# amcpherson/remixt

Measured on AMD Instinct MI355X. Metric: EM iterations/sec (50k seg x 165 states), higher is better.
Workload: dtype f64

## Files before the change

include/remixt_amd.h:

```cpp
#ifndef REMIXT_AMD_H
#define REMIXT_AMD_H

#include <stdint.h>

#ifdef __cplusplus
extern "C" {
#endif

#define RMX_OK 0
#define RMX_EVALUE 1
#define RMX_EASSERT 2
#define RMX_EDEVICE 3
#define RMX_EUNSUPPORTED 4
#define RMX_EARG 5

#define RMX_MAX_CLONES 4

typedef struct rmx_batch rmx_batch;

typedef struct rmx_problem {
    int32_t num_clones;
    int32_t num_segments;
    int32_t num_breakpoints;
    int32_t num_cn_states;
// ... 57 lines not shown
    RMX_OPT_VITERBI_PLAIN,
    RMX_OPT_SEARCH_MODE,
    RMX_OPT_ELL_DENSE,
    RMX_OPT_STRIP,
    RMX_OPT_CELL_CACHE,
    RMX_OPT_SPARSE_TRIAL,
    RMX_OPT_FB_DEBUG,
    RMX_OPT_PAIRWISE_KERNEL,
    RMX_OPT_PACE_SWEEPS,
    RMX_OPT_FB_WG_BUDGET,
    RMX_OPT_TRIAL_KERNEL,
    RMX_OPT_GRAD_KERNEL,
    RMX_OPT_STREAM_POOL,
    RMX_OPT_VITERBI_CLUSTER,
    RMX_OPT_TRACEBACK,
    RMX_OPT_COUNT
};
int rmx_set_default_option(int32_t option_id, int32_t value);
int rmx_set_option(rmx_batch *b, int32_t option_id, int32_t value);
int rmx_get_option(rmx_batch *b, int32_t option_id, int32_t *value);

int rmx_set_param(rmx_batch *b, int32_t r, int32_t param_id, double value);
int rmx_get_param(rmx_batch *b, int32_t r, int32_t param_id, double *value);
int rmx_set_transition_model(rmx_batch *b, int32_t model);
int rmx_set_array(rmx_batch *b, int32_t r, int32_t array_id, const void *host_src);
int rmx_get_array(rmx_batch *b, int32_t r, int32_t array_id, void *host_dst);
int rmx_fetch_indicators(rmx_batch *b, int32_t r0, int32_t r1, const double **total, const double **allele);
int rmx_calculate_log_transmat(rmx_batch *b, int32_t r, double *dst);
int rmx_weighted_search(const double *p, int64_t n, const double *u, int32_t k, int64_t *out, int64_t *positive);
int rmx_weighted_sample_round(const double *w, int64_t n, int64_t stride, double norm, const double *u, int32_t k,
// ... 74 lines not shown
```

remixt_amd/bpmodel.py:

```python
import ctypes as C

import numpy as np

from . import _lib

_dp = C.POINTER(C.c_double)
_ip = C.POINTER(C.c_int64)
_i32p = C.POINTER(C.c_int32)

RMX_EVALUE, RMX_EASSERT, RMX_EDEVICE, RMX_EUNSUPPORTED, RMX_EARG = 1, 2, 3, 4, 5

MAX_CLONES = 4
PARAM_IDS = {
    'negbin_r_0': 0, 'negbin_r_1': 1, 'negbin_hdel_mu': 2, 'negbin_hdel_r_0': 3, 'negbin_hdel_r_1': 4,
    'betabin_M_0': 5, 'betabin_M_1': 6, 'betabin_loh_p': 7, 'betabin_loh_M_0': 8, 'betabin_loh_M_1': 9,
    'prior_outlier_total': 10, 'prior_outlier_allele': 11, 'divergence_weight': 12, 'hmm_log_norm_const': 13,
}
ARRAY_IDS = {
    'h': 0, 'p_breakpoint': 1, 'p_allele_swap': 2, 'p_outlier_total': 3, 'p_outlier_allele': 4,
    'posterior_marginals': 5, 'framelogprob': 6, 'total_likelihood_mask': 7, 'allele_likelihood_mask': 8,
    'log_transmat': 9, 'cached_log_transmat': 10, 'joint_posterior_marginals': 11, 'state_sequence': 12,
}
_WRITABLE = {'h', 'p_breakpoint', 'p_allele_swap', 'p_outlier_total', 'p_outlier_allele', 'posterior_marginals',
             'total_likelihood_mask', 'allele_likelihood_mask'}
_STATE_TABLES = {'cn_states_total': 0, 'num_alleles_subclonal': 1, 'is_hdel': 2, 'is_loh': 3}


OPTION_IDS = dict((n, i) for i, n in enumerate((
    'fb_kernel', 'fb_nv', 'fb_breakend_codes', 'fuse_sweeps', 'two_streams', 'viterbi_plain', 'search_mode', 'ell_dense', 'strip',
    'cell_cache', 'sparse_trial', 'fb_debug', 'pairwise_kernel', 'pace_sweeps', 'fb_wg_budget', 'trial_kernel', 'grad_kernel', 'stream_pool', 'viterbi_cluster', 'traceback')))


def set_default_option(name, value):
    lib = _lib.load()
    rc = lib.rmx_set_default_option(OPTION_IDS[name], int(value))
    if rc:
        _raise(lib, rc)


def last_error_restarts():
    lib = _lib.load()
    n = lib.rmx_last_error_restarts(None, 0)
    if n <= 0:
        return []
    buf = (C.c_int32 * n)()
# ... 791 lines not shown
```

remixt_amd/csrc/rmx_api.hip:

```cpp
#include <hip/hip_runtime.h>
#include <algorithm>
#include <cmath>
#include <limits>
#include <atomic>
#include <cstdio>
#include <cstring>
#include <functional>
#include <map>
#include <mutex>
#include <string>
#include <vector>
#include <chrono>
#include <cstdlib>
#include <condition_variable>
#include <memory>

#include "rmx_kernels.h"
#include "rmx_host.h"

static thread_local std::string g_err;
static thread_local std::vector<int32_t> g_err_restarts;
static int fail(int code, const std::string &msg) { g_err = msg; g_err_restarts.clear(); return code; }
static int fail_flagged(int code, const std::string &msg) { g_err = msg; return code; }
static inline long long now_ns() { return std::chrono::duration_cast<std::chrono::nanoseconds>(std::chrono::steady_clock::now().time_since_epoch()).count(); }
// ... 21 lines not shown
    StreamPool &p = g_stream_pool[dev & 15];
    std::lock_guard<std::mutex> lk(p.mu);
    std::vector<hipStream_t> &idle = p.idle[role];
    if (!idle.empty()) { *out = idle.front(); idle.erase(idle.begin()); return RMX_OK; }
    if (hipStreamCreateWithFlags(out, hipStreamNonBlocking) != hipSuccess) return RMX_EDEVICE;
    p.created[role]++;
    return RMX_OK;
}
static void pool_release(int dev, int role, hipStream_t s) {
    hipStreamSynchronize(s);
    StreamPool &p = g_stream_pool[dev & 15];
    std::lock_guard<std::mutex> lk(p.mu);
    p.idle[role].push_back(s);
}

static int g_opt_default[RMX_OPT_COUNT] = {0, 0, 1, 1, 1, 0, 5, 0, 1, 1, 1, 0, 0, 0, 0, 0, 0, 1, 0, 0};
static std::mutex g_opt_mu;

struct rmx_batch {
    hipEvent_t ev_pace = nullptr;
    int opt[RMX_OPT_COUNT];
    int device = 0;
    hipStream_t stream = nullptr;
    hipStream_t stream2 = nullptr;
    hipEvent_t ev_fb = nullptr, ev_brk = nullptr;
    bool own_stream = false, pooled_stream = false, pooled_stream2 = false;
    Dev d{};
    int R = 0;
    std::vector<int64_t> cn_classes;
    std::vector<int32_t> seg_class, brk_idx, brk_orient, tclass, brk_slot, be_n;
    std::vector<int64_t> brk_states, is_telomere;
// ... 455 lines not shown
                for (int k = 0; k < 8; k++) b->segc_built[(size_t)q * 8 + k] = b->rp[q].p[ids[k]];
                return true;
            };
            if (!stale(r)) { r++; continue; }
            int e = r + 1;
            while (e < r1 && stale(e)) e++;
            { ProfScope ps(b, KID_SEG_CONST); hipLaunchKernelGGL(k_seg_const, dim3((b->d.N + 255) / 256, e - r), dim3(256), 0, b->stream, b->d, r); }
            for (int i = r; i < e; i++) b->segc_dirty[i] = 0;
            r = e;
        }
    }
    HIPCHK(hipGetLastError());
    return RMX_OK;
}
typedef void (*cells_kernel_t)(Dev, int);
template <int NS> static cells_kernel_t cells_kernel_ns(int mode, int mask, int cache) {
    if (mode == 0) return cache == 2 ? k_cells<NS, 0, CM_ALL, 2> : (cache == 1 ? k_cells<NS, 0, CM_ALL, 1> : k_cells<NS, 0, CM_ALL, 0>);
    if (mode == 1) return cache == 2 ? k_cells<NS, 1, CM_ALL, 2> : k_cells<NS, 1, CM_ALL, 0>;
    if (mode == 3) return k_cells<NS, 3, CM_ALL, 2>;
    if (cache == 2) return k_cells<NS, 2, 31, 2>;
    if (cache == 1) {
        switch (mask) {
        case 1: return k_cells<NS, 2, 1, 1>; case 2: return k_cells<NS, 2, 2, 1>;
        case 3: return k_cells<NS, 2, 3, 1>; case 4: return k_cells<NS, 2, 4, 1>; case 8: return k_cells<NS, 2, 8, 1>;
        case 12: return k_cells<NS, 2, 12, 1>; case 15: return k_cells<NS, 2, 15, 1>; default: return k_cells<NS, 2, 31, 1>;
        }
    }
    switch (mask) {
    case 1: return k_cells<NS, 2, 1, 0>; case 2: return k_cells<NS, 2, 2, 0>;
    case 3: return k_cells<NS, 2, 3, 0>; case 4: return k_cells<NS, 2, 4, 0>; case 8: return k_cells<NS, 2, 8, 0>;
    case 12: return k_cells<NS, 2, 12, 0>; case 15: return k_cells<NS, 2, 15, 0>; default: return k_cells<NS, 2, 31, 0>;
    }
}
static bool use_strip(rmx_batch *b) { return b->d.S > 32 && b->d.S <= 384 && b->opt[RMX_OPT_STRIP]; }
static cells_kernel_t cells_kernel(rmx_batch *b, int mode, int mask, int cache) {
    const int ns = (b->d.S + 63) / 64;
    switch (ns) { case 1: return cells_kernel_ns<1>(mode, mask, cache); case 2: return cells_kernel_ns<2>(mode, mask, cache);
                  case 3: return cells_kernel_ns<3>(mode, mask, cache); case 4: return cells_kernel_ns<4>(mode, mask, cache);
                  case 5: return cells_kernel_ns<5>(mode, mask, cache); default: return cells_kernel_ns<6>(mode, mask, cache); }
}
static dim3 ell_block(rmx_batch *b) { return dim3(std::min(256, ((b->d.S + 63) / 64) * 64)); }
static bool ell_sparse_ok(rmx_batch *b, int n, const int32_t *restarts) {
    if (!b->d.sig_cnt || b->opt[RMX_OPT_ELL_DENSE]) return false;
    for (int i = 0; i < n; i++) if (!b->sig_valid[restarts[i]]) return false;
    return true;
}
static dim3 strip_grid(rmx_batch *b, int nr) { return dim3((b->d.N + 4 * STRIP_RPW - 1) / (4 * STRIP_RPW), nr); }
static int cover_mask(int m) {
    if (m & 16) return 31;
    if ((m & 3) && (m & 12)) return 15;
    if ((m & 3) == 3) return 3;
    if (m & 1) return 1;
    if (m & 2) return 2;
    if ((m & 12) == 12) return 12;
// ... 176 lines not shown
    case RMX_OPT_VITERBI_CLUSTER: return v == 0 || v == 1 || v == 2 || v == 4 || v == 8 || v == 102 || v == 104 || v == 108;
    case RMX_OPT_TRACEBACK: return v == 0 || v == 1;
    case RMX_OPT_VITERBI_PLAIN: return v >= 0 && v <= 2;
    default: return v == 0 || v == 1;
    }
}
int rmx_set_default_option(int32_t id, int32_t value) {
    if (id < 0 || id >= RMX_OPT_COUNT || !option_value_ok(id, value)) return fail(RMX_EARG, "bad option id / value");
    std::lock_guard<std::mutex> lk(g_opt_mu);
    g_opt_default[id] = value;
    return RMX_OK;
}
static void configure_fb(rmx_batch *b);
int rmx_set_option(rmx_batch *b, int32_t id, int32_t value) {
    if (!b || id < 0 || id >= RMX_OPT_COUNT || !option_value_ok(id, value)) return fail(RMX_EARG, "bad option id / value");
    if (id == RMX_OPT_CELL_CACHE || id == RMX_OPT_SPARSE_TRIAL || id == RMX_OPT_FB_DEBUG || id == RMX_OPT_STREAM_POOL) return fail(RMX_EARG, "creation-time option: use rmx_set_default_option before rmx_batch_create");
    BIND(b);
    b->opt[id] = value;
    if (id == RMX_OPT_FB_KERNEL) configure_fb(b);
    return RMX_OK;
}
int rmx_get_option(rmx_batch *b, int32_t id, int32_t *value) {
    if (!b || !value || id < 0 || id >= RMX_OPT_COUNT) return fail(RMX_EARG, "bad option id");
    BIND(b);
    *value = b->opt[id];
    return RMX_OK;
}

int rmx_compress_cn_states(const int64_t *cn_states, int32_t N, int32_t S, int32_t M, int32_t max_classes,
                           int32_t *seg_class_out, int64_t *classes_out, int32_t *num_classes) {
    const int rc = rmxh::compress_cn_states(cn_states, N, S, M, max_classes, seg_class_out, classes_out, num_classes);
// ... 157 lines not shown
        if (M == 4 && d.D <= 21 && d.NBE > 0) {
            b->pe2p = (d.D * d.D * d.D + 1) & ~1;
            DA(pe2_lt, double, (size_t)R * d.NBE * b->pe2p + 2)
        }
    }
    if ((rc = dalloc(b, &b->d_A2, RN * 2)) || (rc = dalloc(b, &b->d_Bv2, RN * 4))) { rmx_batch_destroy(b); return rc; }
    if ((rc = dalloc(b, &b->d_cnpack, (size_t)C * S)) || (rc = dalloc(b, &b->d_cnpack2, (size_t)C * S)) || (rc = dalloc(b, &b->d_totpack, (size_t)C * S)) || (rc = dalloc(b, &b->d_wk, (size_t)std::max(d.TC, 1) * FBK_WKN))) { rmx_batch_destroy(b); return rc; }
    DA(pd_cached, double, BEW) DA(hist, double, BEW) DA(be_jt, double, (size_t)R * d.NBE) DA(be_ja, double, (size_t)R * d.NBE)
    DA(err, uint32_t, R)
#undef DA
    d.lc = nullptr; d.sig_idx = nullptr; d.sig_cnt = nullptr;
    if (S > 32 && S <= 384 && b->opt[RMX_OPT_SPARSE_TRIAL]) {
        uint16_t *pi_ = nullptr; uint8_t *pc_ = nullptr;
        if (dalloc(b, &pi_, RN * RMX_SIGK) == RMX_OK && dalloc(b, &pc_, RN) == RMX_OK) { d.sig_idx = pi_; d.sig_cnt = pc_; }
    }
    {
        const size_t bytes = RNS * 6 * 8;
        const bool want = b->opt[RMX_OPT_CELL_CACHE] != 0;
        if (want && S > 32 && S <= 384 && bytes <= ((size_t)96 << 30)) { double *p_ = nullptr; if (dalloc(b, &p_, RNS * 6) == RMX_OK) { d.lc = p_; b->use_cache = true; } }
    }
    if ((rc = dalloc(b, &b->d_lt_valid, R)) || (rc = dalloc(b, &b->d_partial, (size_t)R * ELBO_BLOCKS * 5)) || (rc = dalloc(b, &b->d_be_e, (size_t)R * std::max(d.NBE, 1))) || (rc = dalloc(b, &b->d_out4, (size_t)R * 5)) ||
        (rc = dalloc(b, &b->d_ell_partial, (size_t)R * std::max(N, ELBO_BLOCKS) * (1 + RMX_MAX_CLONES))) || (rc = dalloc(b, &b->d_ell_out, (size_t)R * 8)) ||
        (rc = dalloc(b, &b->d_sample, (size_t)R * N)) || (rc = dalloc(b, &b->d_grid_out, (size_t)R * 64 * (1 + RMX_MAX_CLONES))) ||
        (rc = dalloc(b, &b->d_done, std::max(R, 64))) || (rc = dalloc(b, &b->d_rlist, R)) || (rc = dalloc(b, &b->d_counts, R)) || (rc = dalloc(b, &b->d_rp_stage, R)) || (rc = dalloc(b, &b->d_batch_out, (size_t)R * 8))) { rmx_batch_destroy(b); return rc; }
    HIPCHK(hipMemset(b->d_done, 0, sizeof(unsigned) * (size_t)std::max(R, 64)));
    HIPCHK(hipHostMalloc((void **)&b->h_pinned, sizeof(double) * (size_t)(R + 1) * 64 * (1 + RMX_MAX_CLONES)));
    HIPCHK(hipHostMalloc((void **)&b->h_err, sizeof(uint32_t) * ((size_t)R * 4 + 64)));
    HIPCHK(hipHostMalloc(&b->h_batch, (size_t)R * (sizeof(RestartParams) + 64) + 4096));
    HIPCHK(hipEventCreate(&b->tm_a)); HIPCHK(hipEventCreate(&b->tm_b));
    b->done_ev.resize(R);
    for (int r = 0; r < R; r++) HIPCHK(hipEventCreateWithFlags(&b->done_ev[r], hipEventDisableTiming));

    if ((rc = build_transitions(b))) { rmx_batch_destroy(b); return rc; }
    {
// ... 85 lines not shown
    if (b->own_stream) { if (b->pooled_stream) pool_release(b->device, 0, b->stream); else hipStreamDestroy(b->stream); b->own_stream = false; b->pooled_stream = false; }
    if (s) b->stream = (hipStream_t)s;
    else { HIPCHK(hipStreamCreateWithFlags(&b->stream, hipStreamNonBlocking)); b->own_stream = true; }
    return RMX_OK;
}
int rmx_synchronize(rmx_batch *b) { BIND(b); HIPCHK(hipStreamSynchronize(b->stream)); return RMX_OK; }

int rmx_info(rmx_batch *b, int32_t what, int64_t *out) { BIND(b);
    switch (what) {
    case 0: *out = b->d.cn_max; break; case 1: *out = b->d.NC; break; case 2: *out = b->d.TC; break; case 3: *out = b->d.NBE; break;
    case 4: *out = b->d.SP; break; case 5: *out = b->fbv_rpt; break; case 6: *out = b->fbG.P; break; case 7: *out = b->fbG.NT; break;
    case 8: *out = b->fbG.BLK; break; case 9: *out = (int64_t)b->fbG_lds; break; case 10: *out = b->n_fast; break; case 11: *out = b->n_generic; break;
    case 60: *out = b->t_launch_ns; break; case 61: *out = b->t_wait_ns; break; case 62: *out = b->t_post_ns; break; case 63: *out = b->n_rounds; break;
    case 12: *out = b->last_fb_kernel; break; case 13: *out = b->last_fb_nv; break; case 14: *out = b->last_viterbi; break; case 15: *out = b->last_fb_nv_max; break;
    case 18: *out = b->last_viterbi_wgs; break; case 19: *out = b->last_traceback; break;
    case 54: *out = b->cluster_timeouts; break;
    case 52: *out = b->last_search_blocks; break;
    case 16: { StreamPool &p_ = g_stream_pool[b->device & 15]; std::lock_guard<std::mutex> lk(p_.mu); *out = p_.created[0] + p_.created[1]; break; }
    case 17: { StreamPool &p_ = g_stream_pool[b->device & 15]; std::lock_guard<std::mutex> lk(p_.mu); *out = (int64_t)(p_.idle[0].size() + p_.idle[1].size()); break; }
    case 20: case 21: case 22: case 23: case 24: case 25: case 26: case 27: case 28: case 29: case 30: case 31: case 32: case 33: case 34: case 35: case 36: case 37: case 38: case 39:
    case 40: case 41: case 42: case 43: case 44: case 45: case 46: case 47: case 48: case 49: case 50: case 51:
        { if (!b->d_dbg) { *out = 0; break; } unsigned long long v[32]; HIPCHK(hipStreamSynchronize(b->stream)); HIPCHK(hipMemcpy(v, b->d_dbg, 256, hipMemcpyDeviceToHost)); *out = (int64_t)v[what - 20]; break; }
    default: return fail(RMX_EARG, "bad info id");
    }
    return RMX_OK;
}

static const int kParamComponents[RMX_P_HMM_LOG_NORM_CONST] = {CM_LT0, CM_LT1, CM_LT0 | CM_LT1, CM_LT0, CM_LT1, CM_LA0, CM_LA1, CM_LA0 | CM_LA1, CM_LA0, CM_LA1, 0, 0, 16};
int rmx_set_param(rmx_batch *b, int32_t r, int32_t id, double v) { BIND(b);
    if (r < 0 || r >= b->R || id < 0 || id >= RMX_P_HMM_LOG_NORM_CONST) return fail(RMX_EARG, "bad restart / param id");
// ... 1253 lines not shown
    for (int i = 0; i < nr; i++) out[i] = b->h_pinned[i];
    return RMX_OK;
}

static int trial_pass(rmx_batch *b, int r0, int r1, Dev &d2) {
    b->trial_comp_r0 = b->trial_comp_r1 = -1;
    b->scratch_r0 = b->scratch_r1 = -1;
    int rc = ensure_tables(b, r0, r1);
    if (rc) return rc;
    const Dev &d = b->d;
    const int nr = r1 - r0;
    const size_t RN0 = (size_t)r0 * d.N, cnt = (size_t)nr * d.N;
    HIPCHK(hipMemcpyAsync(b->d_A2 + RN0 * 2, d.A + RN0 * 2, cnt * 16, hipMemcpyDeviceToDevice, b->stream));
    HIPCHK(hipMemcpyAsync(b->d_Bv2 + RN0 * 4, d.Bv + RN0 * 4, cnt * 32, hipMemcpyDeviceToDevice, b->stream));
    d2 = b->d;
    d2.A = b->d_A2; d2.Bv = b->d_Bv2; d2.lc = nullptr;
    for (int r = r0; r < r1;) {
        const int mask = use_strip(b) ? cover_mask(b->comp_dirty[r] & 15) : (b->comp_dirty[r] ? 15 : 0);
        int e = r + 1;
        while (e < r1 && (use_strip(b) ? cover_mask(b->comp_dirty[e] & 15) : (b->comp_dirty[e] ? 15 : 0)) == mask) e++;
        if (mask) {
            ProfScope ps(b, KID_MARGINALS_AB);
            bool sparse = use_strip(b) && d.sig_cnt != nullptr;
            for (int i = r; i < e; i++) if (!b->sig_valid[i]) sparse = false;
            if (sparse) {
                void (*kf)(Dev, int) = nullptr;
                if (b->opt[RMX_OPT_TRIAL_KERNEL] == 0) {
                    switch (mask) {
                    case 1: kf = k_trial_flat<1>; break; case 2: kf = k_trial_flat<2>; break; case 3: kf = k_trial_flat<3>; break;
                    case 4: kf = k_trial_flat<4>; break; case 8: kf = k_trial_flat<8>; break; case 12: kf = k_trial_flat<12>; break;
                    default: kf = k_trial_flat<15>; break;
// ... 559 lines not shown
```

remixt_amd/csrc/rmx_device.h:

```cpp
#pragma once
#include <hip/hip_runtime.h>
#include <stdint.h>
#include "../../include/remixt_amd.h"

#define RMX_ERR_NAN_LL 1u
#define RMX_ERR_BAD_P 2u
#define RMX_ERR_TOTAL_DEPTH 4u
#define RMX_ERR_LOH_P 8u
#define RMX_ERR_NAN_F 16u
#define RMX_ERR_NAN_AB 32u
#define RMX_ERR_NAN_POST 64u
#define RMX_ERR_DIGAMMA 128u
#define RMX_ERR_NAN_GRAD 256u

#define ST_HDEL_NB 1u
#define ST_LOH_M 2u
#define ST_E_TD 4u
#define ST_E_LOH 8u
#define ST_E_BADP 16u
#define ST_GZ_ALLELE 32u

struct RestartParams {
    double h[RMX_MAX_CLONES];
    double p[RMX_P_COUNT];
// ... 26 lines not shown
    const int8_t *af, *ab;
    const uint16_t *pcode;
    const int32_t *jord, *jmeta;
    RestartParams *rp;
    double *stD, *stP, *stM, *stLg;
    double *stLogD;
    uint32_t *stFlags;
    uint32_t *stFlagsAgg;
    double *segc;
    double *qt, *qa, *qs;
    double *pbrk;
    double *f, *fe, *fa, *fb, *post;
    double *fe_alt;
    uint16_t *sig_idx; uint8_t *sig_cnt;
    double *lc;
    double *fmax, *mrow;
    double *A, *Bv;
    double *rowPF, *rowPP, *rowZ;
    double *pd_lt, *pd_cached;
    double *pe_lt;
    double *pe2_lt;
    double *pe2x_lt;
    double *hist;
    double *be_jt, *be_ja;
    uint32_t *err;
};

__device__ __forceinline__ size_t rs_off(const Dev &d, int r, int n) { return ((size_t)r * d.N + n) * d.SP; }

__device__ __forceinline__ double g_transition(int tmodel, int cn_diff) {
// ... 339 lines not shown
```

remixt_amd/csrc/rmx_host.h:

```cpp
#ifndef RMX_HOST_H
#define RMX_HOST_H
#include <algorithm>
#include <cmath>
#include <cstdint>
#include <cstring>
#include <vector>

#if defined(__HIPCC__)
#define RMX_HD __host__ __device__
#else
#define RMX_HD
#endif

namespace rmxh {

inline int compress_cn_states(const int64_t *cn_states, int32_t N, int32_t S, int32_t M, int32_t max_classes,
                              int32_t *seg_class_out, int64_t *classes_out, int32_t *num_classes) {
    if (!cn_states || !seg_class_out || !classes_out || !num_classes) return 5;
    const size_t tsz = (size_t)S * M * 2;
    int C = 0;
    for (int n = 0; n < N; n++) {
        const int64_t *t = cn_states + (size_t)n * tsz;
        int found = -1;
        if (n > 0 && memcmp(t, classes_out + (size_t)seg_class_out[n - 1] * tsz, tsz * 8) == 0) found = seg_class_out[n - 1];
        for (int c = 0; c < C && found < 0; c++) if (memcmp(t, classes_out + (size_t)c * tsz, tsz * 8) == 0) found = c;
        if (found < 0) {
            if (C >= max_classes) return 4;
            memcpy(classes_out + (size_t)C * tsz, t, tsz * 8);
            found = C++;
        }
        seg_class_out[n] = found;
    }
    *num_classes = C;
    return 0;
}

inline int weighted_search(const double *p, int64_t n, const double *u, int32_t k, int64_t *out, int64_t *positive) {
    if (!p || n < 1 || (k > 0 && (!u || !out))) return 5;
    std::vector<double> cdf((size_t)n);
    double acc = 0.;
    int64_t pos = 0;
    for (int64_t i = 0; i < n; i++) { acc += p[i]; cdf[(size_t)i] = acc; pos += p[i] > 0.; }
    const double last = cdf[(size_t)n - 1];
    for (int64_t i = 0; i < n; i++) cdf[(size_t)i] /= last;
    for (int32_t j = 0; j < k; j++) {
        const int64_t idx = (int64_t)(std::upper_bound(cdf.begin(), cdf.end(), u[j]) - cdf.begin());
        out[j] = std::min<int64_t>(idx, n - 1);
    }
// ... 111 lines not shown
```

remixt_amd/csrc/rmx_kernels.h:

```cpp
#pragma once
#include "rmx_device.h"
#include "rmx_host.h"
#define SEGL 32
#define SEG_PER_BLOCK (256 / SEGL)
#define TRIAL_SEGL 16
#define RMX_CLUSTER_SPINS (1u << 22)
#define FBK_WKN 128
#define NM_MAX_SAMPLE 1024
#define TRIAL_SEG_PER_BLOCK (256 / TRIAL_SEGL)


__device__ __forceinline__ void state_tables_body(const Dev &d, int cls, int r, const RestartParams &rp) {
    __shared__ unsigned agg_sh;
    if (threadIdx.x == 0) agg_sh = 0u;
    __syncthreads();
    unsigned agg = 0u;
    for (int s = threadIdx.x; s < d.S; s += blockDim.x) {
        const int8_t *cn = d.cn + ((size_t)cls * d.S + s) * d.M * 2;
        const int8_t *tot = d.tot + ((size_t)cls * d.S + s) * d.M;
        double minor = 0., total = 0.;
        for (int m = 0; m < d.M; m++) {
            minor += rp.h[m] * (double)cn[m * 2 + 0];
            total += rp.h[m] * (double)tot[m];
        }
// ... 1588 lines not shown
    }
    a0 = group_sum(a0, G); a1 = group_sum(a1, G);
    b0 = group_sum(b0, G); b1 = group_sum(b1, G); b2 = group_sum(b2, G); b3 = group_sum(b3, G);
    pf = group_sum(pf, G); pp = group_sum(pp, G);
    if (gl == 0) {
        const size_t rn = (size_t)r * d.N + n;
        d.A[rn * 2] = a0; d.A[rn * 2 + 1] = a1;
        d.Bv[rn * 4] = b0; d.Bv[rn * 4 + 1] = b1; d.Bv[rn * 4 + 2] = b2; d.Bv[rn * 4 + 3] = b3;
        d.rowPF[rn] = pf; d.rowPP[rn] = pp;
        if (COMPUTE_POST) d.rowZ[rn] = d.fmax[rn] + (d.chain_end_flag[n] ? log(sum) : log(d.mrow[rn]));
    }
    if (err) atomicOr(&d.err[r], err);
}

#define STRIP_RPW 8
template <int NS, int MODE, int MASK, int CACHE>
__global__ __launch_bounds__(256) void k_cells(Dev d, int r0) {
    const int r = r0 + blockIdx.y;
    const int lane = threadIdx.x & 63;
    const int wave = __builtin_amdgcn_readfirstlane((int)(threadIdx.x >> 6));
    const int nbeg = (blockIdx.x * 4 + wave) * STRIP_RPW;
    if (nbeg >= d.N) return;
    const int nend = min(d.N, nbeg + STRIP_RPW);
    const RestartParams &rp = d.rp[r];
    const int S = d.S;
    StateRegs st[NS];
    int cur_cls = -1;
    auto nsub_of = [&](int cls_, int s_) { return (double)((d.sflags[(size_t)cls_ * d.S + s_] >> 2) & 3); };
    unsigned err = 0;
    const double divw = rp.p[RMX_P_DIVERGENCE_WEIGHT];
    const size_t plane = (size_t)d.N * d.SP;
    double *lcr = d.lc ? d.lc + (size_t)r * 6 * plane : nullptr;
    auto cell = [&](const SegCtx &sc, const StateRegs &stx, size_t off, double LT[2], double LA[4]) {
        if (CACHE == 2) {
            LT[0] = lcr[off]; LT[1] = lcr[plane + off];
            LA[0] = lcr[2 * plane + off]; LA[1] = lcr[3 * plane + off]; LA[2] = lcr[4 * plane + off]; LA[3] = lcr[5 * plane + off];
        } else {
            cell_ll_regs<MASK & CM_ALL>(rp, sc, stx, LT, LA, err);
            if (CACHE == 1) {
                if (MASK & CM_LT0) lcr[off] = LT[0];
                if (MASK & CM_LT1) lcr[plane + off] = LT[1];
                if (MASK & CM_LA0) { lcr[2 * plane + off] = LA[0]; lcr[3 * plane + off] = LA[1]; }
                if (MASK & CM_LA1) { lcr[4 * plane + off] = LA[2]; lcr[5 * plane + off] = LA[3]; }
            }
        }
    };
    double lp_prior[4] = {0., 0., 0., 0.};
    if (MODE == 3) {
        const double pt_ = rp.p[RMX_P_PRIOR_OUTLIER_TOTAL], pa_ = rp.p[RMX_P_PRIOR_OUTLIER_ALLELE];
        lp_prior[0] = log_prior(1. - pt_); lp_prior[1] = log_prior(pt_); lp_prior[2] = log_prior(1. - pa_); lp_prior[3] = log_prior(pa_);
    }
    constexpr bool PREFETCH = (MODE == 1 || MODE == 3) && NS >= 2 && NS <= 4;
    double pfa[PREFETCH ? NS : 1], pfb[PREFETCH ? NS : 1];
    if (PREFETCH) {
        const size_t ro0 = ((size_t)r * d.N + nbeg) * d.SP;
#pragma unroll
        for (int k = 0; k < NS; k++) { const int s = lane + 64 * k; pfa[k] = s < S ? d.fa[ro0 + s] : 0.; pfb[k] = s < S ? d.fb[ro0 + s] : 0.; }
    }
    for (int n = nbeg; n < nend; n++) {
        const int cls = d.seg_class[n];
        if (CACHE != 2 && cls != cur_cls) {
#pragma unroll
            for (int k = 0; k < NS; k++) { const int s = lane + 64 * k; load_state_regs(d, r, cls, s < S ? s : S - 1, st[k]); }
            cur_cls = cls;
        }
        SegCtx sc; load_seg(d, r, n, sc);
        const size_t rn = (size_t)r * d.N + n;
        const size_t ro = rn * d.SP;
        if (MODE == 0) {
            const double qt0 = d.qt[rn * 2], qt1 = d.qt[rn * 2 + 1], qa0 = d.qa[rn * 2], qa1 = d.qa[rn * 2 + 1];
            const double qs0 = d.qs[rn * 2], qs1 = d.qs[rn * 2 + 1];
            double fv[NS];
            double vmax = -INFINITY;
#pragma unroll
            for (int k = 0; k < NS; k++) {
                const int s = lane + 64 * k;
                fv[k] = -INFINITY;
                if (s < S) {
                    double LT[2], LA[4];
                    cell(sc, st[k], (size_t)n * d.SP + s, LT, LA);
                    double f = 0.;
                    f += qt0 * LT[0]; f += qt1 * LT[1];
                    f += qa0 * qs0 * LA[0]; f += qa0 * qs1 * LA[1]; f += qa1 * qs0 * LA[2]; f += qa1 * qs1 * LA[3];
                    f += -1.0 * (CACHE == 2 ? nsub_of(cls, s) : st[k].nsub) * sc.l * divw;
                    if (f != f) err |= RMX_ERR_NAN_F;
                    d.f[ro + s] = f;
                    fv[k] = f;
                    vmax = fmax(vmax, f);
                }
                __builtin_amdgcn_sched_barrier(0);
            }
            vmax = group_max(vmax, 64);
            if (lane == 0) d.fmax[rn] = vmax;
#pragma unroll
            for (int k = 0; k < NS; k++) { const int s = lane + 64 * k; if (s < d.SP) d.fe[ro + s] = s < S ? exp_fast(fv[k] - vmax) : 0.; }
        } else {
            constexpr bool M1 = MODE == 1 || MODE == 3;
            constexpr int NSTASH = MODE != 3 ? 0 : (NS <= 3 ? 6 : (NS <= 6 ? 3 : 0));
            constexpr bool STASH = NSTASH > 0;
            __shared__ double lsm[STASH ? 4 : 1][STASH ? NS * NSTASH * 64 : 1];
            double pv[NS];
            double sum = 0.;
            if (M1) {
#pragma unroll
                for (int k = 0; k < NS; k++) {
                    const int s = lane + 64 * k;
                    pv[k] = PREFETCH ? pfa[PREFETCH ? k : 0] * pfb[PREFETCH ? k : 0] : (s < S ? d.fa[ro + s] * d.fb[ro + s] : 0.);
                    sum += pv[k];
                }
                if (PREFETCH && n + 1 < nend) {
#pragma unroll
                    for (int k = 0; k < NS; k++) { const int s = lane + 64 * k; pfa[PREFETCH ? k : 0] = s < S ? d.fa[ro + d.SP + s] : 0.; pfb[PREFETCH ? k : 0] = s < S ? d.fb[ro + d.SP + s] : 0.; }
                }
// ... 13 lines not shown
                        const bool sg_ = s < S && pv[k] >= RMX_POST_EPS;
                        const unsigned long long bal_ = __ballot(sg_);
                        const int pos_ = base_ + __popcll(bal_ & ((1ull << lane) - 1ull));
                        if (sg_ && pos_ < RMX_SIGK) d.sig_idx[rn * RMX_SIGK + pos_] = (uint16_t)s;
                        base_ += __popcll(bal_);
                    }
                    if (lane == 0) d.sig_cnt[rn] = base_ <= RMX_SIGK ? (uint8_t)base_ : (uint8_t)255;
                }
            } else {
#pragma unroll
                for (int k = 0; k < NS; k++) { const int s = lane + 64 * k; pv[k] = s < S ? d.post[ro + s] : 0.; }
            }
            double a0 = 0., a1 = 0., b0 = 0., b1 = 0., b2 = 0., b3 = 0., pf = 0., pp = 0.;
            double fq[6] = {0., 0., 0., 0., 0., 0.};
            if (MODE == 1) { fq[0] = d.qt[rn * 2]; fq[1] = d.qt[rn * 2 + 1]; fq[2] = d.qa[rn * 2]; fq[3] = d.qa[rn * 2 + 1]; fq[4] = d.qs[rn * 2]; fq[5] = d.qs[rn * 2 + 1]; }
#pragma unroll
            for (int k = 0; k < NS; k++) {
                const int s = lane + 64 * k;
                if (MODE == 2 && CACHE == 0 && !(MASK & 16) && !__any(pv[k] >= RMX_POST_EPS)) { if (s < S) cell_static_errors<MASK & CM_ALL>(sc, st[k].fl, err); continue; }
                if (s < S) {
                    double LT[2], LA[4];
                    cell(sc, st[k], (size_t)n * d.SP + s, LT, LA);
                    const double ps = pv[k];
                    if (STASH) {
#pragma unroll
                        for (int q_ = 0; q_ < 2; q_++) if (q_ < NSTASH) lsm[wave][(k * NSTASH + q_) * 64 + lane] = LT[q_];
#pragma unroll
                        for (int q_ = 0; q_ < 4; q_++) if (2 + q_ < NSTASH) lsm[wave][(k * NSTASH + 2 + q_) * 64 + lane] = LA[q_];
                    }
                    a0 += ps * LT[0]; a1 += ps * LT[1];
                    b0 += ps * LA[0]; b1 += ps * LA[1]; b2 += ps * LA[2]; b3 += ps * LA[3];
                    if (MODE == 1) {
                        double f = 0.;
                        f += fq[0] * LT[0]; f += fq[1] * LT[1];
                        f += fq[2] * fq[4] * LA[0]; f += fq[2] * fq[5] * LA[1]; f += fq[3] * fq[4] * LA[2]; f += fq[3] * fq[5] * LA[3];
                        f += -1.0 * (CACHE == 2 ? nsub_of(cls, s) : st[k].nsub) * sc.l * divw;
                        d.f[ro + s] = f;
                        pf += ps * f;
                    }
                    if (MODE == 2 && (MASK & 16)) pf += ps * d.f[ro + s];
                    if (MODE == 1 || (MODE == 2 && (MASK & 16))) pp += ps * (-1.0 * (CACHE == 2 ? nsub_of(cls, s) : st[k].nsub) * sc.l * divw);
                }
                __builtin_amdgcn_sched_barrier(0);
// ... 39 lines not shown
                { const double ss_ = qs0 + qs1; qs0 /= ss_; qs1 /= ss_; }
                if (lane == 0) {
                    d.qt[rn * 2] = qt0; d.qt[rn * 2 + 1] = qt1; d.qa[rn * 2] = qa0; d.qa[rn * 2 + 1] = qa1;
                    d.qs[rn * 2] = qs0; d.qs[rn * 2 + 1] = qs1;
                }
                double fv[NS];
                double vmax = -INFINITY;
#pragma unroll
                for (int k = 0; k < NS; k++) {
                    const int s = lane + 64 * k;
                    fv[k] = -INFINITY;
                    if (s < S) {
                        double LT[2], LA[4];
                        if (STASH) {
                            const size_t off_ = (size_t)n * d.SP + s;
#pragma unroll
                            for (int q_ = 0; q_ < 2; q_++) LT[q_] = q_ < NSTASH ? lsm[wave][(k * NSTASH + q_) * 64 + lane] : lcr[q_ * plane + off_];
#pragma unroll
                            for (int q_ = 0; q_ < 4; q_++) LA[q_] = 2 + q_ < NSTASH ? lsm[wave][(k * NSTASH + 2 + q_) * 64 + lane] : lcr[(2 + q_) * plane + off_];
                        } else cell(sc, st[k], (size_t)n * d.SP + s, LT, LA);
                        double f = 0.;
                        f += qt0 * LT[0]; f += qt1 * LT[1];
                        f += qa0 * qs0 * LA[0]; f += qa0 * qs1 * LA[1]; f += qa1 * qs0 * LA[2]; f += qa1 * qs1 * LA[3];
                        f += -1.0 * nsub_of(cls, s) * sc.l * divw;
                        if (f != f) err |= RMX_ERR_NAN_F;
                        fv[k] = f;
                        vmax = fmax(vmax, f);
                    }
                }
                vmax = group_max(vmax, 64);
                if (lane == 0) d.fmax[rn] = vmax;
#pragma unroll
                for (int k = 0; k < NS; k++) { const int s = lane + 64 * k; if (s < d.SP) d.fe_alt[ro + s] = s < S ? exp_fast(fv[k] - vmax) : 0.; }
            }
        }
// ... 3181 lines not shown
```

Baseline: 449.0.

## Cache total-likelihood terms per distinct total-copy-number class instead of per state

States that share the same total copy number per clone (and the same homozygous-deletion flag) give identical total-read likelihoods. A host pass groups states into these classes per segment class. When the cell cache is built, the kernel computes the two total-likelihood planes only once per representative state, stores them in a compact per-segment array and broadcasts them through LDS using packed per-lane class indices. This cuts total-likelihood arithmetic and cache memory and traffic from six planes to four plus a small class table. It adds a wave barrier, LDS use and extra template variants, and falls back when there are more than 128 classes.

```diff
diff --git a/include/remixt_amd.h b/include/remixt_amd.h
--- a/include/remixt_amd.h
+++ b/include/remixt_amd.h
@@ -95,6 +95,7 @@
     RMX_OPT_STREAM_POOL,
     RMX_OPT_VITERBI_CLUSTER,
     RMX_OPT_TRACEBACK,
+    RMX_OPT_LT_CLASSES,
     RMX_OPT_COUNT
 };
 int rmx_set_default_option(int32_t option_id, int32_t value);
diff --git a/remixt_amd/bpmodel.py b/remixt_amd/bpmodel.py
--- a/remixt_amd/bpmodel.py
+++ b/remixt_amd/bpmodel.py
@@ -28,7 +28,7 @@
 
 OPTION_IDS = dict((n, i) for i, n in enumerate((
     'fb_kernel', 'fb_nv', 'fb_breakend_codes', 'fuse_sweeps', 'two_streams', 'viterbi_plain', 'search_mode', 'ell_dense', 'strip',
-    'cell_cache', 'sparse_trial', 'fb_debug', 'pairwise_kernel', 'pace_sweeps', 'fb_wg_budget', 'trial_kernel', 'grad_kernel', 'stream_pool', 'viterbi_cluster', 'traceback')))
+    'cell_cache', 'sparse_trial', 'fb_debug', 'pairwise_kernel', 'pace_sweeps', 'fb_wg_budget', 'trial_kernel', 'grad_kernel', 'stream_pool', 'viterbi_cluster', 'traceback', 'lt_classes')))
 
 
 def set_default_option(name, value):
diff --git a/remixt_amd/csrc/rmx_api.hip b/remixt_amd/csrc/rmx_api.hip
--- a/remixt_amd/csrc/rmx_api.hip
+++ b/remixt_amd/csrc/rmx_api.hip
@@ -59,7 +59,7 @@
     p.idle[role].push_back(s);
 }
 
-static int g_opt_default[RMX_OPT_COUNT] = {0, 0, 1, 1, 1, 0, 5, 0, 1, 1, 1, 0, 0, 0, 0, 0, 0, 1, 0, 0};
+static int g_opt_default[RMX_OPT_COUNT] = {0, 0, 1, 1, 1, 0, 5, 0, 1, 1, 1, 0, 0, 0, 0, 0, 0, 1, 0, 0, 1};
 static std::mutex g_opt_mu;
 
 struct rmx_batch {
@@ -545,30 +545,34 @@
     return RMX_OK;
 }
 typedef void (*cells_kernel_t)(Dev, int);
-template <int NS> static cells_kernel_t cells_kernel_ns(int mode, int mask, int cache) {
-    if (mode == 0) return cache == 2 ? k_cells<NS, 0, CM_ALL, 2> : (cache == 1 ? k_cells<NS, 0, CM_ALL, 1> : k_cells<NS, 0, CM_ALL, 0>);
-    if (mode == 1) return cache == 2 ? k_cells<NS, 1, CM_ALL, 2> : k_cells<NS, 1, CM_ALL, 0>;
-    if (mode == 3) return k_cells<NS, 3, CM_ALL, 2>;
-    if (cache == 2) return k_cells<NS, 2, 31, 2>;
-    if (cache == 1) {
-        switch (mask) {
-        case 1: return k_cells<NS, 2, 1, 1>; case 2: return k_cells<NS, 2, 2, 1>;
-        case 3: return k_cells<NS, 2, 3, 1>; case 4: return k_cells<NS, 2, 4, 1>; case 8: return k_cells<NS, 2, 8, 1>;
-        case 12: return k_cells<NS, 2, 12, 1>; case 15: return k_cells<NS, 2, 15, 1>; default: return k_cells<NS, 2, 31, 1>;
-        }
-    }
+template <int NS, int LTC> static cells_kernel_t cells_kernel_cached(int mode, int mask, int cache) {
+    if (mode == 0) return cache == 2 ? k_cells<NS, 0, CM_ALL, 2, LTC> : k_cells<NS, 0, CM_ALL, 1, LTC>;
+    if (mode == 1) return k_cells<NS, 1, CM_ALL, 2, LTC>;
+    if (mode == 3) return k_cells<NS, 3, CM_ALL, 2, LTC>;
+    if (cache == 2) return k_cells<NS, 2, 31, 2, LTC>;
     switch (mask) {
-    case 1: return k_cells<NS, 2, 1, 0>; case 2: return k_cells<NS, 2, 2, 0>;
-    case 3: return k_cells<NS, 2, 3, 0>; case 4: return k_cells<NS, 2, 4, 0>; case 8: return k_cells<NS, 2, 8, 0>;
-    case 12: return k_cells<NS, 2, 12, 0>; case 15: return k_cells<NS, 2, 15, 0>; default: return k_cells<NS, 2, 31, 0>;
+    case 1: return k_cells<NS, 2, 1, 1, LTC>; case 2: return k_cells<NS, 2, 2, 1, LTC>;
+    case 3: return k_cells<NS, 2, 3, 1, LTC>; case 4: return k_cells<NS, 2, 4, 1, LTC>; case 8: return k_cells<NS, 2, 8, 1, LTC>;
+    case 12: return k_cells<NS, 2, 12, 1, LTC>; case 15: return k_cells<NS, 2, 15, 1, LTC>; default: return k_cells<NS, 2, 31, 1, LTC>;
+    }
+}
+template <int NS> static cells_kernel_t cells_kernel_ns(int mode, int mask, int cache, bool ltc) {
+    if (cache) return ltc ? cells_kernel_cached<NS, 1>(mode, mask, cache) : cells_kernel_cached<NS, 0>(mode, mask, cache);
+    if (mode == 0) return k_cells<NS, 0, CM_ALL, 0, 0>;
+    if (mode == 1) return k_cells<NS, 1, CM_ALL, 0, 0>;
+    switch (mask) {
+    case 1: return k_cells<NS, 2, 1, 0, 0>; case 2: return k_cells<NS, 2, 2, 0, 0>;
+    case 3: return k_cells<NS, 2, 3, 0, 0>; case 4: return k_cells<NS, 2, 4, 0, 0>; case 8: return k_cells<NS, 2, 8, 0, 0>;
+    case 12: return k_cells<NS, 2, 12, 0, 0>; case 15: return k_cells<NS, 2, 15, 0, 0>; default: return k_cells<NS, 2, 31, 0, 0>;
     }
 }
 static bool use_strip(rmx_batch *b) { return b->d.S > 32 && b->d.S <= 384 && b->opt[RMX_OPT_STRIP]; }
 static cells_kernel_t cells_kernel(rmx_batch *b, int mode, int mask, int cache) {
     const int ns = (b->d.S + 63) / 64;
-    switch (ns) { case 1: return cells_kernel_ns<1>(mode, mask, cache); case 2: return cells_kernel_ns<2>(mode, mask, cache);
-                  case 3: return cells_kernel_ns<3>(mode, mask, cache); case 4: return cells_kernel_ns<4>(mode, mask, cache);
-                  case 5: return cells_kernel_ns<5>(mode, mask, cache); default: return cells_kernel_ns<6>(mode, mask, cache); }
+    const bool ltc = cache != 0 && b->d.ltc != nullptr;
+    switch (ns) { case 1: return cells_kernel_ns<1>(mode, mask, cache, ltc); case 2: return cells_kernel_ns<2>(mode, mask, cache, ltc);
+                  case 3: return cells_kernel_ns<3>(mode, mask, cache, ltc); case 4: return cells_kernel_ns<4>(mode, mask, cache, ltc);
+                  case 5: return cells_kernel_ns<5>(mode, mask, cache, ltc); default: return cells_kernel_ns<6>(mode, mask, cache, ltc); }
 }
 static dim3 ell_block(rmx_batch *b) { return dim3(std::min(256, ((b->d.S + 63) / 64) * 64)); }
 static bool ell_sparse_ok(rmx_batch *b, int n, const int32_t *restarts) {
@@ -775,7 +779,7 @@
 static void configure_fb(rmx_batch *b);
 int rmx_set_option(rmx_batch *b, int32_t id, int32_t value) {
     if (!b || id < 0 || id >= RMX_OPT_COUNT || !option_value_ok(id, value)) return fail(RMX_EARG, "bad option id / value");
-    if (id == RMX_OPT_CELL_CACHE || id == RMX_OPT_SPARSE_TRIAL || id == RMX_OPT_FB_DEBUG || id == RMX_OPT_STREAM_POOL) return fail(RMX_EARG, "creation-time option: use rmx_set_default_option before rmx_batch_create");
+    if (id == RMX_OPT_CELL_CACHE || id == RMX_OPT_SPARSE_TRIAL || id == RMX_OPT_FB_DEBUG || id == RMX_OPT_STREAM_POOL || id == RMX_OPT_LT_CLASSES) return fail(RMX_EARG, "creation-time option: use rmx_set_default_option before rmx_batch_create");
     BIND(b);
     b->opt[id] = value;
     if (id == RMX_OPT_FB_KERNEL) configure_fb(b);
@@ -963,10 +967,27 @@
         uint16_t *pi_ = nullptr; uint8_t *pc_ = nullptr;
         if (dalloc(b, &pi_, RN * RMX_SIGK) == RMX_OK && dalloc(b, &pc_, RN) == RMX_OK) { d.sig_idx = pi_; d.sig_cnt = pc_; }
     }
+    d.ltc = nullptr; d.ltcls = nullptr; d.ltrep = nullptr; d.NT = 0; d.NTP = 0;
     {
+        std::vector<int32_t> cls_, rep_, cnt_;
+        int32_t nt_ = 0;
+        if (rmxh::lt_classes(b->cn_classes.data(), C, S, M, cls_, rep_, cnt_, &nt_)) { rmx_batch_destroy(b); return fail(RMX_EARG, "bad state tables"); }
+        d.NT = nt_; d.NTP = ((nt_ + 7) / 8) * 8;
+        const bool compact = b->opt[RMX_OPT_LT_CLASSES] != 0 && nt_ <= 128;
         const size_t bytes = RNS * 6 * 8;
         const bool want = b->opt[RMX_OPT_CELL_CACHE] != 0;
-        if (want && S > 32 && S <= 384 && bytes <= ((size_t)96 << 30)) { double *p_ = nullptr; if (dalloc(b, &p_, RNS * 6) == RMX_OK) { d.lc = p_; b->use_cache = true; } }
+        if (want && S > 32 && S <= 384 && bytes <= ((size_t)96 << 30)) {
+            double *p_ = nullptr, *q_ = nullptr;
+            if (!compact) { if (dalloc(b, &p_, RNS * 6) == RMX_OK) { d.lc = p_; b->use_cache = true; } }
+            else {
+                std::vector<uint8_t> cls8((size_t)C * S);
+                std::vector<int32_t> rep((size_t)C * d.NTP, 0);
+                for (size_t i = 0; i < cls8.size(); i++) cls8[i] = (uint8_t)cls_[i];
+                for (int c = 0; c < C; c++) for (int k = 0; k < cnt_[c]; k++) rep[(size_t)c * d.NTP + k] = rep_[(size_t)c * S + k];
+                if (dalloc(b, &p_, RNS * 4) == RMX_OK && dalloc(b, &q_, RN * d.NTP * 2) == RMX_OK &&
+                    dupload(b, &d.ltcls, cls8) == RMX_OK && dupload(b, &d.ltrep, rep) == RMX_OK) { d.lc = p_; d.ltc = q_; b->use_cache = true; }
+            }
+        }
     }
     if ((rc = dalloc(b, &b->d_lt_valid, R)) || (rc = dalloc(b, &b->d_partial, (size_t)R * ELBO_BLOCKS * 5)) || (rc = dalloc(b, &b->d_be_e, (size_t)R * std::max(d.NBE, 1))) || (rc = dalloc(b, &b->d_out4, (size_t)R * 5)) ||
         (rc = dalloc(b, &b->d_ell_partial, (size_t)R * std::max(N, ELBO_BLOCKS) * (1 + RMX_MAX_CLONES))) || (rc = dalloc(b, &b->d_ell_out, (size_t)R * 8)) ||
@@ -1082,6 +1103,7 @@
     case 60: *out = b->t_launch_ns; break; case 61: *out = b->t_wait_ns; break; case 62: *out = b->t_post_ns; break; case 63: *out = b->n_rounds; break;
     case 12: *out = b->last_fb_kernel; break; case 13: *out = b->last_fb_nv; break; case 14: *out = b->last_viterbi; break; case 15: *out = b->last_fb_nv_max; break;
     case 18: *out = b->last_viterbi_wgs; break; case 19: *out = b->last_traceback; break;
+    case 64: *out = b->d.NT; break; case 65: *out = b->d.ltc ? 1 : 0; break;
     case 54: *out = b->cluster_timeouts; break;
     case 52: *out = b->last_search_blocks; break;
     case 16: { StreamPool &p_ = g_stream_pool[b->device & 15]; std::lock_guard<std::mutex> lk(p_.mu); *out = p_.created[0] + p_.created[1]; break; }
@@ -2365,7 +2387,7 @@
     HIPCHK(hipMemcpyAsync(b->d_A2 + RN0 * 2, d.A + RN0 * 2, cnt * 16, hipMemcpyDeviceToDevice, b->stream));
     HIPCHK(hipMemcpyAsync(b->d_Bv2 + RN0 * 4, d.Bv + RN0 * 4, cnt * 32, hipMemcpyDeviceToDevice, b->stream));
     d2 = b->d;
-    d2.A = b->d_A2; d2.Bv = b->d_Bv2; d2.lc = nullptr;
+    d2.A = b->d_A2; d2.Bv = b->d_Bv2; d2.lc = nullptr; d2.ltc = nullptr;
     for (int r = r0; r < r1;) {
         const int mask = use_strip(b) ? cover_mask(b->comp_dirty[r] & 15) : (b->comp_dirty[r] ? 15 : 0);
         int e = r + 1;
diff --git a/remixt_amd/csrc/rmx_device.h b/remixt_amd/csrc/rmx_device.h
--- a/remixt_amd/csrc/rmx_device.h
+++ b/remixt_amd/csrc/rmx_device.h
@@ -64,6 +64,10 @@
     double *fe_alt;
     uint16_t *sig_idx; uint8_t *sig_cnt;
     double *lc;
+    double *ltc;
+    const uint8_t *ltcls;
+    const int32_t *ltrep;
+    int NT, NTP;
     double *fmax, *mrow;
     double *A, *Bv;
     double *rowPF, *rowPP, *rowZ;
diff --git a/remixt_amd/csrc/rmx_host.h b/remixt_amd/csrc/rmx_host.h
--- a/remixt_amd/csrc/rmx_host.h
+++ b/remixt_amd/csrc/rmx_host.h
@@ -32,6 +32,31 @@
         seg_class_out[n] = found;
     }
     *num_classes = C;
+    return 0;
+}
+
+inline int lt_classes(const int64_t *cn_classes, int32_t C, int32_t S, int32_t M,
+                      std::vector<int32_t> &ltcls, std::vector<int32_t> &ltrep, std::vector<int32_t> &count, int32_t *NT) {
+    if (!cn_classes || !NT || C < 1 || S < 1 || M < 1) return 5;
+    ltcls.assign((size_t)C * S, -1); ltrep.assign((size_t)C * S, -1); count.assign((size_t)C, 0);
+    std::vector<int64_t> keys((size_t)S * (M + 1)), key((size_t)M + 1);
+    int32_t nt = 0;
+    for (int c = 0; c < C; c++) {
+        int k = 0;
+        for (int s = 0; s < S; s++) {
+            const int64_t *t = cn_classes + ((size_t)c * S + s) * M * 2;
+            bool hdel = true;
+            for (int m = 0; m < M; m++) { key[(size_t)m] = t[m * 2] + t[m * 2 + 1]; if (t[m * 2] != 0 || t[m * 2 + 1] != 0) hdel = false; }
+            key[(size_t)M] = hdel ? 1 : 0;
+            int found = -1;
+            for (int j = 0; j < k && found < 0; j++) if (std::equal(key.begin(), key.end(), keys.begin() + (size_t)j * (M + 1))) found = j;
+            if (found < 0) { std::copy(key.begin(), key.end(), keys.begin() + (size_t)k * (M + 1)); ltrep[(size_t)c * S + k] = s; found = k++; }
+            ltcls[(size_t)c * S + s] = found;
+        }
+        count[(size_t)c] = k;
+        nt = std::max(nt, (int32_t)k);
+    }
+    *NT = nt;
     return 0;
 }
 
diff --git a/remixt_amd/csrc/rmx_kernels.h b/remixt_amd/csrc/rmx_kernels.h
--- a/remixt_amd/csrc/rmx_kernels.h
+++ b/remixt_amd/csrc/rmx_kernels.h
@@ -1626,8 +1626,9 @@
 }
 
 #define STRIP_RPW 8
-template <int NS, int MODE, int MASK, int CACHE>
+template <int NS, int MODE, int MASK, int CACHE, int LTC>
 __global__ __launch_bounds__(256) void k_cells(Dev d, int r0) {
+    static_assert(!LTC || CACHE != 0, "class rows belong to the cell cache");
     const int r = r0 + blockIdx.y;
     const int lane = threadIdx.x & 63;
     const int wave = __builtin_amdgcn_readfirstlane((int)(threadIdx.x >> 6));
@@ -1642,18 +1643,34 @@
     unsigned err = 0;
     const double divw = rp.p[RMX_P_DIVERGENCE_WEIGHT];
     const size_t plane = (size_t)d.N * d.SP;
-    double *lcr = d.lc ? d.lc + (size_t)r * 6 * plane : nullptr;
-    auto cell = [&](const SegCtx &sc, const StateRegs &stx, size_t off, double LT[2], double LA[4]) {
+    double *lcr = d.lc ? d.lc + (size_t)r * (LTC ? 4 : 6) * plane : nullptr;
+    double *lar = lcr ? lcr + (LTC ? 0 : 2) * plane : nullptr;
+    constexpr bool LTG0 = LTC && (CACHE == 2 || (MASK & CM_LT0)), LTG1 = LTC && (CACHE == 2 || (MASK & CM_LT1));
+    constexpr bool LTG = LTG0 || LTG1;
+    const size_t lplane = LTC ? (size_t)d.N * d.NTP : 0;
+    double *ltr = LTC ? d.ltc + (size_t)r * 2 * lplane : nullptr;
+    __shared__ double ltl[LTC ? 4 : 1][LTC ? 256 : 1];
+    unsigned ci_lo = 0, ci_hi = 0;
+    double repD[LTG && CACHE == 1 ? 2 : 1] = {}, repLogD[LTG && CACHE == 1 ? 2 : 1] = {};
+    unsigned repFl[LTG && CACHE == 1 ? 2 : 1] = {};
+    auto lt_gather = [&](int k, double LT[2]) {
+        const unsigned c_ = ((k < 4 ? ci_lo : ci_hi) >> (8 * (k & 3))) & 0xffu;
+        LT[0] = LTG0 ? ltl[wave][c_] : 0.;
+        LT[1] = LTG1 ? ltl[wave][128 + c_] : 0.;
+    };
+    auto cell = [&](const SegCtx &sc, const StateRegs &stx, size_t off, int k, double LT[2], double LA[4]) {
         if (CACHE == 2) {
-            LT[0] = lcr[off]; LT[1] = lcr[plane + off];
-            LA[0] = lcr[2 * plane + off]; LA[1] = lcr[3 * plane + off]; LA[2] = lcr[4 * plane + off]; LA[3] = lcr[5 * plane + off];
+            if (LTC) lt_gather(k, LT);
+            else { LT[0] = lcr[off]; LT[1] = lcr[plane + off]; }
+            LA[0] = lar[off]; LA[1] = lar[plane + off]; LA[2] = lar[2 * plane + off]; LA[3] = lar[3 * plane + off];
         } else {
-            cell_ll_regs<MASK & CM_ALL>(rp, sc, stx, LT, LA, err);
+            cell_ll_regs<LTC ? (MASK & (CM_LA0 | CM_LA1)) : (MASK & CM_ALL)>(rp, sc, stx, LT, LA, err);
+            if (LTC) lt_gather(k, LT);
             if (CACHE == 1) {
-                if (MASK & CM_LT0) lcr[off] = LT[0];
-                if (MASK & CM_LT1) lcr[plane + off] = LT[1];
-                if (MASK & CM_LA0) { lcr[2 * plane + off] = LA[0]; lcr[3 * plane + off] = LA[1]; }
-                if (MASK & CM_LA1) { lcr[4 * plane + off] = LA[2]; lcr[5 * plane + off] = LA[3]; }
+                if (!LTC && (MASK & CM_LT0)) lcr[off] = LT[0];
+                if (!LTC && (MASK & CM_LT1)) lcr[plane + off] = LT[1];
+                if (MASK & CM_LA0) { lar[off] = LA[0]; lar[plane + off] = LA[1]; }
+                if (MASK & CM_LA1) { lar[2 * plane + off] = LA[2]; lar[3 * plane + off] = LA[3]; }
             }
         }
     };
@@ -1671,26 +1688,72 @@
     }
     for (int n = nbeg; n < nend; n++) {
         const int cls = d.seg_class[n];
-        if (CACHE != 2 && cls != cur_cls) {
-#pragma unroll
-            for (int k = 0; k < NS; k++) { const int s = lane + 64 * k; load_state_regs(d, r, cls, s < S ? s : S - 1, st[k]); }
+        if ((CACHE != 2 || LTG) && cls != cur_cls) {
+            if (CACHE != 2) {
+#pragma unroll
+                for (int k = 0; k < NS; k++) { const int s = lane + 64 * k; load_state_regs(d, r, cls, s < S ? s : S - 1, st[k]); }
+            }
+            if (LTG) {
+                ci_lo = 0u; ci_hi = 0u;
+#pragma unroll
+                for (int k = 0; k < NS; k++) {
+                    const int s = lane + 64 * k;
+                    const unsigned c_ = d.ltcls[(size_t)cls * S + (s < S ? s : S - 1)];
+                    if (k < 4) ci_lo |= c_ << (8 * (k & 3)); else ci_hi |= c_ << (8 * (k & 3));
+                }
+                if (CACHE == 1) {
+#pragma unroll
+                    for (int j = 0; j < 2; j++) {
+                        const int kc = lane + 64 * j;
+                        if (kc < d.NT) {
+                            const size_t si = ((size_t)r * d.C + cls) * d.SP + d.ltrep[(size_t)cls * d.NTP + kc];
+                            repD[LTG && CACHE == 1 ? j : 0] = d.stD[si]; repLogD[LTG && CACHE == 1 ? j : 0] = d.stLogD[si]; repFl[LTG && CACHE == 1 ? j : 0] = d.stFlags[si];
+                        }
+                    }
+                }
+            }
             cur_cls = cls;
         }
         SegCtx sc; load_seg(d, r, n, sc);
         const size_t rn = (size_t)r * d.N + n;
         const size_t ro = rn * d.SP;
+        double ltq0 = 0., ltq1 = 0.;
+        if (LTG && CACHE == 2 && lane < d.NT) { ltq0 = ltr[(size_t)n * d.NTP + lane]; ltq1 = ltr[lplane + (size_t)n * d.NTP + lane]; }
+        auto lt_rows_to_lds = [&]() {
+            if (!LTG) return;
+            const size_t lo_ = (size_t)n * d.NTP;
+            if (CACHE == 2) {
+                if (lane < d.NT) { ltl[wave][lane] = ltq0; ltl[wave][128 + lane] = ltq1; }
+                if (d.NT > 64 && lane + 64 < d.NT) { ltl[wave][64 + lane] = ltr[lo_ + 64 + lane]; ltl[wave][192 + lane] = ltr[lplane + lo_ + 64 + lane]; }
+            } else {
+#pragma unroll
+                for (int j = 0; j < 2; j++) {
+                    const int kc = lane + 64 * j;
+                    if ((j == 0 || d.NT > 64) && kc < d.NT) {
+                        StateRegs rs_ = {};
+                        rs_.D = repD[LTG && CACHE == 1 ? j : 0]; rs_.logD = repLogD[LTG && CACHE == 1 ? j : 0]; rs_.fl = repFl[LTG && CACHE == 1 ? j : 0];
+                        double LTc[2], LAc[4];
+                        cell_ll_regs<MASK & (CM_LT0 | CM_LT1)>(rp, sc, rs_, LTc, LAc, err);
+                        if (LTG0) { ltr[lo_ + kc] = LTc[0]; ltl[wave][kc] = LTc[0]; }
+                        if (LTG1) { ltr[lplane + lo_ + kc] = LTc[1]; ltl[wave][128 + kc] = LTc[1]; }
+                    }
+                }
+            }
+            __builtin_amdgcn_wave_barrier();
+        };
         if (MODE == 0) {
             const double qt0 = d.qt[rn * 2], qt1 = d.qt[rn * 2 + 1], qa0 = d.qa[rn * 2], qa1 = d.qa[rn * 2 + 1];
             const double qs0 = d.qs[rn * 2], qs1 = d.qs[rn * 2 + 1];
             double fv[NS];
             double vmax = -INFINITY;
+            lt_rows_to_lds();
 #pragma unroll
             for (int k = 0; k < NS; k++) {
                 const int s = lane + 64 * k;
                 fv[k] = -INFINITY;
                 if (s < S) {
                     double LT[2], LA[4];
-                    cell(sc, st[k], (size_t)n * d.SP + s, LT, LA);
+                    cell(sc, st[k], (size_t)n * d.SP + s, k, LT, LA);
                     double f = 0.;
                     f += qt0 * LT[0]; f += qt1 * LT[1];
                     f += qa0 * qs0 * LA[0]; f += qa0 * qs1 * LA[1]; f += qa1 * qs0 * LA[2]; f += qa1 * qs1 * LA[3];
@@ -1708,7 +1771,8 @@
             for (int k = 0; k < NS; k++) { const int s = lane + 64 * k; if (s < d.SP) d.fe[ro + s] = s < S ? exp_fast(fv[k] - vmax) : 0.; }
         } else {
             constexpr bool M1 = MODE == 1 || MODE == 3;
-            constexpr int NSTASH = MODE != 3 ? 0 : (NS <= 3 ? 6 : (NS <= 6 ? 3 : 0));
+            constexpr int LAOFF = LTC ? 0 : 2;
+            constexpr int NSTASH = MODE != 3 ? 0 : LTC ? (NS <= 3 ? 4 : (NS == 4 ? 3 : 2)) : (NS <= 3 ? 6 : (NS <= 6 ? 3 : 0));
             constexpr bool STASH = NSTASH > 0;
             __shared__ double lsm[STASH ? 4 : 1][STASH ? NS * NSTASH * 64 : 1];
             double pv[NS];
@@ -1752,19 +1816,20 @@
             double a0 = 0., a1 = 0., b0 = 0., b1 = 0., b2 = 0., b3 = 0., pf = 0., pp = 0.;
             double fq[6] = {0., 0., 0., 0., 0., 0.};
             if (MODE == 1) { fq[0] = d.qt[rn * 2]; fq[1] = d.qt[rn * 2 + 1]; fq[2] = d.qa[rn * 2]; fq[3] = d.qa[rn * 2 + 1]; fq[4] = d.qs[rn * 2]; fq[5] = d.qs[rn * 2 + 1]; }
+            lt_rows_to_lds();
 #pragma unroll
             for (int k = 0; k < NS; k++) {
                 const int s = lane + 64 * k;
                 if (MODE == 2 && CACHE == 0 && !(MASK & 16) && !__any(pv[k] >= RMX_POST_EPS)) { if (s < S) cell_static_errors<MASK & CM_ALL>(sc, st[k].fl, err); continue; }
                 if (s < S) {
                     double LT[2], LA[4];
-                    cell(sc, st[k], (size_t)n * d.SP + s, LT, LA);
+                    cell(sc, st[k], (size_t)n * d.SP + s, k, LT, LA);
                     const double ps = pv[k];
                     if (STASH) {
 #pragma unroll
-                        for (int q_ = 0; q_ < 2; q_++) if (q_ < NSTASH) lsm[wave][(k * NSTASH + q_) * 64 + lane] = LT[q_];
-#pragma unroll
-                        for (int q_ = 0; q_ < 4; q_++) if (2 + q_ < NSTASH) lsm[wave][(k * NSTASH + 2 + q_) * 64 + lane] = LA[q_];
+                        for (int q_ = 0; q_ < 2; q_++) if (!LTC && q_ < NSTASH) lsm[wave][(k * NSTASH + q_) * 64 + lane] = LT[q_];
+#pragma unroll
+                        for (int q_ = 0; q_ < 4; q_++) if (LAOFF + q_ < NSTASH) lsm[wave][(k * NSTASH + LAOFF + q_) * 64 + lane] = LA[q_];
                     }
                     a0 += ps * LT[0]; a1 += ps * LT[1];
                     b0 += ps * LA[0]; b1 += ps * LA[1]; b2 += ps * LA[2]; b3 += ps * LA[3];
@@ -1834,11 +1899,14 @@
                         double LT[2], LA[4];
                         if (STASH) {
                             const size_t off_ = (size_t)n * d.SP + s;
-#pragma unroll
-                            for (int q_ = 0; q_ < 2; q_++) LT[q_] = q_ < NSTASH ? lsm[wave][(k * NSTASH + q_) * 64 + lane] : lcr[q_ * plane + off_];
-#pragma unroll
-                            for (int q_ = 0; q_ < 4; q_++) LA[q_] = 2 + q_ < NSTASH ? lsm[wave][(k * NSTASH + 2 + q_) * 64 + lane] : lcr[(2 + q_) * plane + off_];
-                        } else cell(sc, st[k], (size_t)n * d.SP + s, LT, LA);
+                            if (LTC) lt_gather(k, LT);
+                            else {
+#pragma unroll
+                                for (int q_ = 0; q_ < 2; q_++) LT[q_] = q_ < NSTASH ? lsm[wave][(k * NSTASH + q_) * 64 + lane] : lcr[q_ * plane + off_];
+                            }
+#pragma unroll
+                            for (int q_ = 0; q_ < 4; q_++) LA[q_] = LAOFF + q_ < NSTASH ? lsm[wave][(k * NSTASH + LAOFF + q_) * 64 + lane] : lar[q_ * plane + off_];
+                        } else cell(sc, st[k], (size_t)n * d.SP + s, k, LT, LA);
                         double f = 0.;
                         f += qt0 * LT[0]; f += qt1 * LT[1];
                         f += qa0 * qs0 * LA[0]; f += qa0 * qs1 * LA[1]; f += qa1 * qs0 * LA[2]; f += qa1 * qs1 * LA[3];
```

New measurement: 454.0, median of 6. +1.1%, better.
